# lh3/miniasm

Hardware: AMD Instinct MI355X
Metric: PAF overlaps processed/sec (hit-filter->trans-reduce->GFA) (higher is better)
Workload: dtype u32

## Files before the change

include/mahip.h:

```cpp
#ifndef MAHIP_H
#define MAHIP_H

#include <stddef.h>
#include <stdint.h>
#include "miniasm_amd.h"

#ifdef __cplusplus
extern "C" {
#endif

typedef struct mahip_ctx mahip_ctx_t;

int mahip_device_count(void);
mahip_ctx_t *mahip_create(int device, void *stream);
void mahip_destroy(mahip_ctx_t *c);
const char *mahip_strerror(void);
int mahip_sync(mahip_ctx_t *c);
int mahip_first_launch(mahip_ctx_t *c);

int mahip_hits_upload(mahip_ctx_t *c, const ma_hit_t *h, size_t n, uint32_t n_seq);
int mahip_hits_adopt(mahip_ctx_t *c, const void *d_hits, size_t n, uint32_t n_seq);
int mahip_set_shard(mahip_ctx_t *c, uint32_t q_beg, uint32_t q_end);
int mahip_hits_balance(mahip_ctx_t *c, int world, uint32_t *bounds);
int mahip_set_shard_bounds(mahip_ctx_t *c, const uint32_t *bounds, int world);
// ... 114 lines not shown
int mahip_map_download(mahip_ctx_t *c, int32_t *map);
uint32_t mahip_n_seq_new(mahip_ctx_t *c);
int mahip_survivors_download(mahip_ctx_t *c, uint32_t *old_ids);
size_t mahip_hits_live(mahip_ctx_t *c);
int mahip_hits_download(mahip_ctx_t *c, ma_hit_t *out, size_t *n);

int mahip_sg_gen(mahip_ctx_t *c, const ma_opt_t *opt, int use_sub, const uint32_t *seq_len, const uint8_t *seq_del, uint32_t *n_arc);
int mahip_asg_upload(mahip_ctx_t *c, const asg_t *g);
int mahip_asg_del_trans(mahip_ctx_t *c, int fuzz, uint32_t *n_reduced);
int mahip_asg_symm(mahip_ctx_t *c, uint32_t *n_multi, uint32_t *n_asymm);
int mahip_asg_del_multi(mahip_ctx_t *c, uint32_t *n_multi);
int mahip_asg_del_asymm(mahip_ctx_t *c, uint32_t *n_asymm);
int mahip_asg_del_short(mahip_ctx_t *c, float drop_ratio, uint32_t *n_short);
int mahip_asg_squeeze(mahip_ctx_t *c);
int mahip_tail_handoff(mahip_ctx_t *from, mahip_ctx_t *to);
int mahip_asg_cut_tip(mahip_ctx_t *c, int max_ext, uint32_t *n_cut);
int mahip_asg_cut_internal(mahip_ctx_t *c, int max_ext, uint32_t *n_cut);
int mahip_asg_cut_biloop(mahip_ctx_t *c, int max_ext, uint32_t *n_cut);
int mahip_asg_pop_bubble(mahip_ctx_t *c, int max_dist, uint32_t *n_pop, uint32_t *n_tips);
uint32_t mahip_bubble_seq_sweeps(mahip_ctx_t *c);
enum { MAHIP_BUBBLE_TIERS = 5, MAHIP_BUBBLE_THREAD = 1, MAHIP_BUBBLE_WAVE_LDS = 2, MAHIP_BUBBLE_WAVE_HBM = 3 };
typedef struct { uint32_t n_iter, max_tier, seq_sweep, form[MAHIP_BUBBLE_TIERS]; uint64_t n_src[MAHIP_BUBBLE_TIERS]; } mahip_clean_info_t;
int mahip_clean_last(mahip_ctx_t *c, mahip_clean_info_t *out);
int mahip_ug_gen(mahip_ctx_t *c, uint32_t *n_utg, uint32_t *n_members, uint32_t *n_uarc);
int mahip_ug_download(mahip_ctx_t *c, uint32_t *u_n, uint32_t *u_len, uint32_t *u_start, uint32_t *u_end, uint32_t *u_off, uint64_t *members, asg_arc_t *uarcs);
typedef struct { uint64_t src_off, dst_off; uint32_t src_len, len; uint32_t rev, pad; } mahip_useq_job_t;
int mahip_useq_begin(mahip_ctx_t *c, size_t arena_bytes);
int mahip_useq_batch(mahip_ctx_t *c, const char *h_seq, size_t seq_bytes, const mahip_useq_job_t *h_jobs, size_t n_jobs);
int mahip_useq_end(mahip_ctx_t *c, char *h_arena);
enum { MAHIP_FASTX_OK = 0, MAHIP_FASTX_CR, MAHIP_FASTX_FIRST_BYTE, MAHIP_FASTX_FASTA_LINE_START, MAHIP_FASTX_FASTQ_SHAPE, MAHIP_FASTX_FASTQ_QUAL_LEN, MAHIP_FASTX_TOO_MANY_LINES,
// ... 268 lines not shown
```

miniasm_amd/csrc/graph.hip:

```cpp
#include "mahip_internal.hpp"
#include <type_traits>

#define DEAD 0x80000000u
#define ADEL 0x80000000u

struct HitColsG { const uint32_t *qid, *qs, *qe, *tn, *ts, *te, *ml, *bl; };
struct ArcCols { uint32_t *u, *v, *len, *ol; };

static HitColsG gcols_of(mahip_ctx *c)
{
	HitColsG h;
	h.qid = P<uint32_t>(c->col[0]); h.qs = P<uint32_t>(c->col[1]); h.qe = P<uint32_t>(c->col[2]); h.tn = P<uint32_t>(c->col[3]);
	h.ts = P<uint32_t>(c->col[4]); h.te = P<uint32_t>(c->col[5]); h.ml = P<uint32_t>(c->col[6]); h.bl = P<uint32_t>(c->col[7]);
	return h;
}
static ArcCols arcs_of(mahip_ctx *c, int g)
{
	ArcCols a;
	a.u = P<uint32_t>(c->au[g]); a.v = P<uint32_t>(c->av[g]); a.len = P<uint32_t>(c->alen[g]); a.ol = P<uint32_t>(c->aol[g]);
	return a;
}
static int reserve_arcs(mahip_ctx *c, size_t n)
{
	for (int g = 0; g < 2; ++g) {
// ... 897 lines not shown
	c->n_arc = n_out;
	c->arcs_clean = true;
	if (index_mode > 0 || (index_mode == 0 && changed)) CHK(arc_reindex(c));
	return 0;
}


extern "C" int mahip_sg_flags(mahip_ctx_t *c, const ma_opt_t *opt, int use_sub, const uint32_t *seq_len, const uint8_t *seq_del)
{
	HIPCHK(hipSetDevice(c->dev));
	CHK(hits_need_cols(c, "mahip_sg_gen"));
	size_t n = c->n_hits;
	uint32_t R = c->n_seq;
	CHK(dev_reserve(c, c->slen, ((size_t)R + 4) * 4)); CHK(dev_reserve(c, c->sdel, (size_t)R + 16));
	c->sg_max_hang = opt->max_hang; c->sg_int_frac = opt->int_frac; c->sg_min_ovlp = opt->min_ovlp;
	c->gsq = false; c->arcs_clean = false;
	CHK(ctr_zero(c));
	unsigned long long *ctr = P<unsigned long long>(c->ctr);
	const uint32_t *d_len = nullptr; const uint8_t *d_del = nullptr;
	if (seq_len) { CHK(dev_reserve(c, c->big0, ((size_t)R + 4) * 4)); HIPCHK(hipMemcpyAsync(c->big0.p, seq_len, (size_t)R * 4, hipMemcpyHostToDevice, c->st)); d_len = P<uint32_t>(c->big0); }
	if (seq_del) { CHK(dev_reserve(c, c->big1, (size_t)R + 16)); HIPCHK(hipMemcpyAsync(c->big1.p, seq_del, R, hipMemcpyHostToDevice, c->st)); d_del = P<uint8_t>(c->big1); }
	if (!use_sub && !d_len) { mahip_set_error("mahip_sg_gen: need sub or seq_len"); return -1; }
	if (R) hipLaunchKernelGGL(k_sg_seq, dim3(grid_for(R, 256)), dim3(256), 0, c->st, use_sub ? (const uint2*)P<uint2>(c->sub[0]) : (const uint2*)nullptr,
	                          c->has_map ? (const uint8_t*)P<uint8_t>(c->r_del) : (const uint8_t*)nullptr, d_len, d_del, R, P<uint32_t>(c->slen), P<uint8_t>(c->sdel));
	c->ag = 0;
	if (n) CHK(dev_reserve(c, c->sgmask, (n / 64 + 8) * 8));
	if (n) {
		ProfScope ps(c, "k_sg_arcs", 64.0 * (double)c->n_live);
		hipLaunchKernelGGL(k_sg_arcs, dim3(grid_for(n, 256, MA_STREAM_BLOCKS)), dim3(256), 0, c->st, gcols_of(c), n, (const uint32_t*)P<uint32_t>(c->slen), P<uint8_t>(c->sdel),
		                   opt->max_hang, opt->int_frac, opt->min_ovlp, ctr,
		                   c->lazy_squeeze ? (const uint8_t*)P<uint8_t>(c->r_del) : (const uint8_t*)nullptr, P<unsigned long long>(c->sgmask));
// ... 376 lines not shown
		HIPCHK(hipMemcpyAsync(c->slen.p, c->big0.p, (size_t)Rn * 4, hipMemcpyDeviceToDevice, c->st));
		HIPCHK(hipMemcpyAsync(c->sdel.p, c->big1.p, (size_t)Rn, hipMemcpyDeviceToDevice, c->st));
		HIPCHK(hipMemcpyAsync(c->idx.p, c->pos.p, 2 * (size_t)Rn * 8, hipMemcpyDeviceToDevice, c->st));
	}
	HIPCHK(hipGetLastError());
	c->gsq = true;
	return 0;
}

__global__ __launch_bounds__(256) void k_sub_squeeze_g(const uint2 *__restrict__ sub, const int32_t *__restrict__ map, uint32_t n_seq, uint2 *__restrict__ out)
{
	uint32_t r = blockIdx.x * 256 + threadIdx.x;
	if (r < n_seq && map[r] >= 0) out[map[r]] = sub[r];
}

extern "C" int mahip_tail_handoff(mahip_ctx_t *s, mahip_ctx_t *d)
{
	if (s == d || s->dev != d->dev) { mahip_set_error("mahip_tail_handoff: two contexts on one device"); return -1; }
	HIPCHK(hipSetDevice(s->dev));
	if (!s->graph_ready) { mahip_set_error("mahip_tail_handoff: no graph"); return -1; }
	CHK(mahip_asg_squeeze(s));
	const uint32_t Rn = s->has_map ? s->n_seq_new : s->n_seq;
	const size_t n = s->n_arc;
	const bool have_sub = s->sub[0].p != nullptr && s->n_seq > 0;
	CHK(reserve_arcs(d, n));
	CHK(dev_reserve(d, d->slen, ((size_t)Rn + 4) * 4)); CHK(dev_reserve(d, d->sdel, (size_t)Rn + 16));
	CHK(dev_reserve(d, d->idx, (2 * (size_t)Rn + 2) * 8));
	CHK(dev_reserve(d, d->sub[0], ((size_t)Rn + 1) * 8)); CHK(dev_reserve(d, d->surv, ((size_t)Rn + 1) * 4));
	if (n) {
		HIPCHK(hipMemcpyAsync(d->au[0].p, s->au[s->ag].p, n * 4, hipMemcpyDeviceToDevice, s->st));
		HIPCHK(hipMemcpyAsync(d->av[0].p, s->av[s->ag].p, n * 4, hipMemcpyDeviceToDevice, s->st));
		HIPCHK(hipMemcpyAsync(d->alen[0].p, s->alen[s->ag].p, n * 4, hipMemcpyDeviceToDevice, s->st));
		HIPCHK(hipMemcpyAsync(d->aol[0].p, s->aol[s->ag].p, n * 4, hipMemcpyDeviceToDevice, s->st));
	}
	if (Rn) {
		HIPCHK(hipMemcpyAsync(d->slen.p, s->slen.p, (size_t)Rn * 4, hipMemcpyDeviceToDevice, s->st));
		HIPCHK(hipMemcpyAsync(d->sdel.p, s->sdel.p, (size_t)Rn, hipMemcpyDeviceToDevice, s->st));
		HIPCHK(hipMemcpyAsync(d->idx.p, s->idx.p, 2 * (size_t)Rn * 8, hipMemcpyDeviceToDevice, s->st));
		if (have_sub) {
			if (s->has_map) hipLaunchKernelGGL(k_sub_squeeze_g, dim3(grid_for(s->n_seq, 256)), dim3(256), 0, s->st, (const uint2*)P<uint2>(s->sub[0]), (const int32_t*)P<int32_t>(s->map), s->n_seq, P<uint2>(d->sub[0]));
			else HIPCHK(hipMemcpyAsync(d->sub[0].p, s->sub[0].p, (size_t)Rn * 8, hipMemcpyDeviceToDevice, s->st));
		}
		if (s->has_map || s->surv_ready) HIPCHK(hipMemcpyAsync(d->surv.p, s->surv.p, (size_t)Rn * 4, hipMemcpyDeviceToDevice, s->st));
	}
	HIPCHK(hipGetLastError());
	HIPCHK(hipStreamSynchronize(s->st));
	d->n_seq = Rn; d->n_seq_new = Rn; d->has_map = false; d->surv_ready = s->has_map || s->surv_ready; d->gsq = true; d->lazy_squeeze = false;
	d->soa_ready = false; d->gather_pending = false; d->sorted_here = false; d->n_hits = 0; d->n_live = 0;
	d->ag = 0; d->n_arc = (uint32_t)n; d->graph_ready = true;
	d->arcs_clean = s->arcs_clean;
	d->tie = s->tie;
	return 0;
}

extern "C" int mahip_asg_cleanup(mahip_ctx_t *c, uint32_t *n_arc)
{
	HIPCHK(hipSetDevice(c->dev));
	if (!c->graph_ready) { mahip_set_error("mahip_asg_cleanup: no graph"); return -1; }
	CHK(ctr_zero(c));
	CHK(arc_cleanup(c, c->n_arc, 0, 0));
	if (n_arc) *n_arc = c->n_arc;
	return 0;
}

// ... 170 lines not shown
```

miniasm_amd/csrc/hits.hip:

```cpp
#include "mahip_internal.hpp"

#define COL_QID 0
#define COL_QS 1
#define COL_QE 2
#define COL_TN 3
#define COL_TS 4
#define COL_TE 5
#define COL_ML 6
#define COL_BL 7
#define DEAD 0x80000000u

__global__ __launch_bounds__(256) void k_hit_keys(const ma_hit_t *__restrict__ h, size_t n, uint64_t *__restrict__ key,
                                                   uint32_t *__restrict__ val, uint32_t *__restrict__ keep, unsigned long long *__restrict__ ctr,
                                                   uint32_t q_beg, uint32_t q_end, int bi, int full)
{
	uint32_t cnt = 0;
	for (size_t i = (size_t)blockIdx.x * 256 + threadIdx.x; i < n; i += (size_t)gridDim.x * 256) {
		uint64_t k = h[i].qns;
		uint32_t q = (uint32_t)(k >> 32);
		int in = q >= q_beg && q < q_end;
		cnt += in;
		if (full) key[i] = k, val[i] = (uint32_t)i;
		else key[i] = (uint64_t)q << bi | i;
		if (keep) keep[i] = in;
// ... 860 lines not shown
static int reserve_read_arrays(mahip_ctx *c)
{
	size_t R = c->n_seq;
	CHK(dev_reserve(c, c->goff, (R + 2) * 4));
	for (int k = 0; k < 2; ++k) CHK(dev_reserve(c, c->sub[k], (R + 1) * 8));
	CHK(dev_reserve(c, c->r_cont, R + 16)); CHK(dev_reserve(c, c->r_used, R + 16));
	CHK(dev_reserve(c, c->r_del, R + 16)); CHK(dev_reserve(c, c->r_live, R + 16));
	CHK(dev_reserve(c, c->map, (R + 1) * 4));
	CHK(dev_reserve(c, c->surv, (R + 1) * 4));
	return 0;
}

static int hits_common_setup(mahip_ctx *c, size_t n, uint32_t n_seq)
{
	c->n_hits = n; c->n_in = n; c->n_live = n; c->n_seq = n_seq; c->n_seq_new = n_seq;
	c->soa_ready = false; c->has_map = false; c->surv_ready = false; c->graph_ready = false; c->gather_pending = false;
	c->hint_max_qs = 0; c->run_stride = 0; c->gk_runs = false; c->n_runs = 0;
	c->lazy_squeeze = false;
	c->sorted_here = false; c->hrank_ready = false; c->orank_ready = false;
	c->n_total = 0;
	c->shard_bounds.clear();
	memset(&c->tie, 0, sizeof(c->tie));
	CHK(reserve_read_arrays(c));
	for (int k = 0; k < 8; ++k) CHK(dev_reserve(c, c->col[k], (n + 128) * 4));
	return 0;
}

extern "C" int mahip_hits_upload(mahip_ctx_t *c, const ma_hit_t *h, size_t n, uint32_t n_seq)
{
	HIPCHK(hipSetDevice(c->dev));
	CHK(hits_common_setup(c, n, n_seq));
// ... 1016 lines not shown
```

miniasm_amd/csrc/mahip_api.hip:

```cpp
#include "mahip_internal.hpp"
#include <stdarg.h>

static thread_local char g_err[1024] = "";

void mahip_set_error(const char *fmt, ...)
{
	va_list ap;
	va_start(ap, fmt);
	vsnprintf(g_err, sizeof(g_err), fmt, ap);
	va_end(ap);
}

extern "C" const char *mahip_strerror(void) { return g_err; }

extern "C" int mahip_device_count(void)
{
	int n = 0;
	if (hipGetDeviceCount(&n) != hipSuccess) return 0;
	return n;
}

static bool pool_on() { static int v = -1; if (v < 0) { const char *e = getenv("MA_DEV_POOL"); v = !(e && atoi(e) == 0); } return v != 0; }

static std::mutex g_reg_mu;
static std::vector<mahip_ctx*> g_ctxs;
static void ctx_register(mahip_ctx *c) { std::lock_guard<std::mutex> g(g_reg_mu); g_ctxs.push_back(c); }
static void ctx_unregister(mahip_ctx *c)
{
	std::lock_guard<std::mutex> g(g_reg_mu);
	for (size_t i = 0; i < g_ctxs.size(); ++i) if (g_ctxs[i] == c) { g_ctxs[i] = g_ctxs.back(); g_ctxs.pop_back(); break; }
}

static DevPool::Base *pool_base_of(DevPool &P, const char *p)
{
	for (DevPool::Base &b : P.bases) if (p >= b.p && p < b.p + b.bytes) return &b;
	return nullptr;
}

static void pool_give_back(mahip_ctx *c, char *p, size_t cap)
{
	DevPool &P = c->pool;
	std::lock_guard<std::mutex> g(P.mu);
	DevPool::Base *base = pool_base_of(P, p);
	if (!base) { (void)hipFree(p); return; }
	DevPool::Piece nw = { p, cap, base->p };
	for (size_t i = 0; i < P.free_pieces.size();) {
		DevPool::Piece &f = P.free_pieces[i];
		if (f.base == nw.base && (f.p + f.cap == nw.p || nw.p + nw.cap == f.p)) {
			if (f.p < nw.p) nw.p = f.p;
			nw.cap += f.cap;
			P.free_pieces[i] = P.free_pieces.back(); P.free_pieces.pop_back();
			i = 0;
		} else ++i;
	}
	P.free_pieces.push_back(nw);
}

static size_t pool_trim_locked(DevPool &P)
{
	size_t freed = 0;
	for (size_t i = 0; i < P.free_pieces.size();) {
		const DevPool::Piece f = P.free_pieces[i];
		DevPool::Base *b = pool_base_of(P, f.p);
		if (b && f.p == b->p && f.cap == b->bytes) {
			(void)hipFree(b->p);
			freed += b->bytes;
			*b = P.bases.back(); P.bases.pop_back();
			P.free_pieces[i] = P.free_pieces.back(); P.free_pieces.pop_back();
		} else ++i;
	}
	return freed;
}
static size_t pool_trim(mahip_ctx *c) { std::lock_guard<std::mutex> g(c->pool.mu); return pool_trim_locked(c->pool); }
static void pool_trim_siblings(mahip_ctx *c)
{
	std::lock_guard<std::mutex> g(g_reg_mu);
	for (mahip_ctx *o : g_ctxs) if (o != c && o->dev == c->dev) (void)pool_trim(o);
}
static size_t pool_idle_bytes(mahip_ctx *c)
{
	std::lock_guard<std::mutex> g(c->pool.mu);
	size_t n = 0;
	for (const DevPool::Piece &f : c->pool.free_pieces) n += f.cap;
	return n;
}

static int pool_take(mahip_ctx *c, size_t want, void **out, size_t *cap)
{
	DevPool &P = c->pool;
	{
		std::lock_guard<std::mutex> g(P.mu);
		size_t best = (size_t)-1;
		for (size_t i = 0; i < P.free_pieces.size(); ++i)
			if (P.free_pieces[i].cap >= want && (best == (size_t)-1 || P.free_pieces[i].cap < P.free_pieces[best].cap)) best = i;
		if (best != (size_t)-1) {
			DevPool::Piece &f = P.free_pieces[best];
			*out = f.p;
			if (f.cap - want >= ((size_t)1 << 20)) { *cap = want; f.p += want; f.cap -= want; }
			else { *cap = f.cap; P.free_pieces[best] = P.free_pieces.back(); P.free_pieces.pop_back(); }
			return 0;
		}
	}
	void *p = nullptr;
	hipError_t e = hipMalloc(&p, want);
	if (e != hipSuccess) { (void)hipGetLastError(); (void)hipStreamSynchronize(c->st); (void)pool_trim(c); e = hipMalloc(&p, want); }
	if (e != hipSuccess) { (void)hipGetLastError(); pool_trim_siblings(c); e = hipMalloc(&p, want); }
	if (e != hipSuccess) { (void)hipGetLastError(); mahip_set_error("hipMalloc(%zu bytes) failed: %s (%zu bytes in use by this context)", want, hipGetErrorString(e), c->mem_bytes); return -1; }
	std::lock_guard<std::mutex> g(P.mu);
	P.bases.push_back({ (char*)p, want });
	*out = p; *cap = want;
	return 0;
}

void dev_pool_destroy(mahip_ctx *c)
{
	std::lock_guard<std::mutex> g(c->pool.mu);
	for (DevPool::Base &b : c->pool.bases) (void)hipFree(b.p);
	c->pool.bases.clear(); c->pool.free_pieces.clear();
}

int dev_reserve(mahip_ctx *c, DevBuf &b, size_t bytes)
{
	if (bytes <= b.cap) return 0;
	if (b.p) { HIPCHK(hipStreamSynchronize(c->st)); dev_free(c, b); }
	size_t want = (bytes + 255) & ~(size_t)255;
	if (pool_on()) {
		if (pool_take(c, want, &b.p, &b.cap) != 0) { b.p = nullptr; b.cap = 0; return -1; }
	} else {
		hipError_t e = hipMalloc(&b.p, want);
		if (e != hipSuccess) { (void)hipGetLastError(); b.p = nullptr; mahip_set_error("hipMalloc(%zu bytes) failed: %s", want, hipGetErrorString(e)); return -1; }
		b.cap = want;
	}
	c->mem_bytes += b.cap;
	return 0;
}

void dev_free(mahip_ctx *c, DevBuf &b)
{
	if (b.p) {
		c->mem_bytes -= b.cap;
		if (pool_on()) {
			if (b.ext) (void)hipDeviceSynchronize();
			pool_give_back(c, (char*)b.p, b.cap);
		} else (void)hipFree(b.p);
	}
	b.p = nullptr; b.cap = 0; b.ext = false;
}

extern "C" int mahip_mem_trim(mahip_ctx_t *c, size_t *released)
{
	HIPCHK(hipSetDevice(c->dev));
	HIPCHK(hipStreamSynchronize(c->st));
	const size_t n = pool_trim(c);
	if (released) *released = n;
	return 0;
}
extern "C" size_t mahip_mem_pool_bytes(mahip_ctx_t *c) { return pool_idle_bytes(c); }

int ctr_zero(mahip_ctx *c)
{
	HIPCHK(hipMemsetAsync(c->ctr.p, 0, CT_STICKY * 8, c->st));
// ... 81 lines not shown
	closedir(dp);
}

extern "C" mahip_ctx_t *mahip_create(int device, void *stream)
{
	int n = 0;
	hipError_t e = hipGetDeviceCount(&n);
	if (e != hipSuccess || n <= 0) {
		mahip_set_error("mahip_create: no HIP device available (%s); this library has no CPU fallback", e == hipSuccess ? "device count 0" : hipGetErrorString(e));
		return nullptr;
	}
	if (device < 0 || device >= n) { mahip_set_error("mahip_create: device %d out of range (0..%d)", device, n - 1); return nullptr; }
	if (hipSetDevice(device) != hipSuccess) { mahip_set_error("mahip_create: hipSetDevice(%d) failed", device); return nullptr; }
	pin_to_gpu_node(device);
	mahip_ctx *c = new mahip_ctx();
	c->dev = device;
	ctx_register(c);
	if (stream) c->st = (hipStream_t)stream, c->own_stream = false;
	else {
		if (hipStreamCreateWithFlags(&c->st, hipStreamNonBlocking) != hipSuccess) { mahip_set_error("mahip_create: hipStreamCreate failed"); ctx_unregister(c); delete c; return nullptr; }
		c->own_stream = true;
	}
	if (dev_reserve(c, c->ctr, CT_ALLOC_WORDS * 8) != 0) { ctx_unregister(c); delete c; return nullptr; }
	if (hipHostMalloc((void**)&c->h_ctr, 72 * 8, hipHostMallocCoherent | hipHostMallocMapped) != hipSuccess) { mahip_set_error("mahip_create: hipHostMalloc failed"); ctx_unregister(c); delete c; return nullptr; }
	memset(c->h_ctr, 0, 72 * 8);
	if (hipMemsetAsync(c->ctr.p, 0, CT_ALLOC_WORDS * 8, c->st) != hipSuccess) { mahip_set_error("mahip_create: memset failed"); ctx_unregister(c); delete c; return nullptr; }
	{ const char *s = getenv("MA_EXACT_TIES"); c->tie_mode = s == 0 || *s == 0 ? 2 : atoi(s) != 0 ? 1 : 0; }
	return c;
}

extern "C" void mahip_destroy(mahip_ctx_t *c)
{
	if (!c) return;
	ctx_unregister(c);
	(void)hipSetDevice(c->dev);
	(void)hipStreamSynchronize(c->st);
	for (auto &e : c->pev) { (void)hipEventDestroy(e.a); (void)hipEventDestroy(e.b); }
	for (hipEvent_t e : c->mark_ev) if (e) (void)hipEventDestroy(e);
	for (hipEvent_t e : c->sub_ev) if (e) (void)hipEventDestroy(e);
	for (hipStream_t t : c->sub_side) if (t) (void)hipStreamDestroy(t);
	DevBuf *all[] = { &c->aos_own, &c->goff, &c->sub[0], &c->sub[1], &c->r_cont, &c->r_used, &c->r_del, &c->r_live, &c->map, &c->surv,
		&c->au[0], &c->au[1], &c->av[0], &c->av[1], &c->alen[0], &c->alen[1], &c->aol[0], &c->aol[1], &c->idx, &c->sdel, &c->slen,
		&c->keep, &c->pos, &c->gs_tmp, &c->key[0], &c->key[1], &c->val[0], &c->val[1], &c->hist, &c->scan_tmp[0], &c->scan_tmp[1], &c->scan_tmp[2],
		&c->ctr, &c->ovf, &c->big0, &c->big1, &c->marks, &c->sgmask, &c->sidx, &c->hrank, &c->orank, &c->aslot, &c->apos, &c->pushrows[0], &c->pushrows[1], &c->xb[0], &c->xb[1], &c->gpos, &c->tdig, &c->wantb, &c->wseg };
	for (DevBuf *b : all) dev_free(c, *b);
	for (int k = 0; k < 8; ++k) dev_free(c, c->col[k]);
	c->hwalk.drop(); c->hdig.drop();
	mahip_comm_destroy(c);
	paf_free(c);
	clean_free(c);
	ug_free(c);
	useq_free(c);
	text_free(c);
	xfer_pool_free(c);
	free(c->gzip_rows);
	free(c->gzip_members);
	dev_pool_destroy(c);
	if (c->h_ctr) (void)hipHostFree(c->h_ctr);
	if (c->own_stream) (void)hipStreamDestroy(c->st);
	delete c;
}
// ... 119 lines not shown
```

miniasm_amd/csrc/mahip_internal.hpp:

```cpp
#pragma once
#include <hip/hip_runtime.h>
#include <stdint.h>
#include <stdio.h>
#include <stdlib.h>
#include <string.h>
#include <time.h>
#include <vector>
#include <mutex>
#include <string>
#include "mahip.h"
#include "ma_core.h"

void mahip_set_error(const char *fmt, ...);
extern "C" int ma_timing_level(void);

#define HIPCHK(expr) do { hipError_t e_ = (expr); if (e_ != hipSuccess) { \
	mahip_set_error("%s:%d: %s -> %s", __FILE__, __LINE__, #expr, hipGetErrorString(e_)); return -1; } } while (0)
#define CHK(expr) do { int r_ = (expr); if (r_ != 0) return r_; } while (0)

struct DevBuf {
	void *p = nullptr;
	size_t cap = 0;
	bool ext = false;
};

struct ProfEvent { const char *name; hipEvent_t a, b; double alg_bytes; };
struct ProfAcc { const char *name; uint64_t launches; double ms; double alg_bytes; };

struct DevPool {
	struct Base { char *p; size_t bytes; };
	struct Piece { char *p; size_t cap; char *base; };
	std::vector<Base> bases;
	std::vector<Piece> free_pieces;
	std::mutex mu;
};

struct BigHost { void *p = nullptr; size_t bytes = 0; bool mapped = false; bool reserve(size_t n); void drop(); };

struct mahip_ctx {
	int dev = 0;
	hipStream_t st = nullptr;
	bool own_stream = false;
	size_t mem_bytes = 0;
	DevPool pool;

	size_t n_hits = 0;
	size_t n_in = 0;
	bool full_input = true;
	DevBuf gpos;
	uint64_t n_total = 0;
	size_t n_live = 0;
	uint32_t n_seq = 0;
	uint32_t q_beg = 0, q_end = 0xffffffffu;
	std::vector<uint32_t> shard_bounds;
	uint32_t hint_max_qs = 0;
	uint32_t paf_max_qs = 0;
	const ma_hit_t *d_aos = nullptr;
	DevBuf aos_own;
	DevBuf col[8];
	DevBuf goff;
	DevBuf sub[2];
	DevBuf r_cont, r_used, r_del, r_live;
	DevBuf map;
	DevBuf surv;
	bool soa_ready = false, has_map = false, lazy_squeeze = false;
	bool surv_ready = false;
	int sg_max_hang = 0, sg_min_ovlp = 0; float sg_int_frac = 0;
	int tie_mode = 2;
	DevBuf sidx;
	DevBuf hrank;
	DevBuf orank;
	DevBuf aslot;
	DevBuf apos;
	DevBuf pushrows[2];
	uint32_t n_push = 0;
	bool sorted_here = false, hrank_ready = false, orank_ready = false;
	bool gather_pending = false; int gk_gen = 0, gk_bi = 0;
	bool gk_runs = false; size_t n_runs = 0; int run_stride = 0;
	bool push_ordered = false;
	mahip_tie_info_t tie = {0, 0, 0, 0, 0, 0, 0, 0, 0};
	uint32_t n_seq_new = 0;

	DevBuf au[2], av[2], alen[2], aol[2];
	int ag = 0;
	uint32_t n_arc = 0;
	DevBuf idx;
	DevBuf sdel;
	DevBuf slen;
	bool graph_ready = false;
	bool gsq = false;
	void *comm = nullptr;
	DevBuf xb[2];
	void *clean = nullptr;
	void *ug = nullptr;
	void *useq = nullptr;
	void *text = nullptr;

	DevBuf keep, pos;
	BigHost hwalk, hdig;
	DevBuf tdig;
	DevBuf wantb;
	DevBuf wseg;
	DevBuf key[2], val[2];
	DevBuf hist;
	DevBuf scan_tmp[3];
	DevBuf gs_tmp;
	DevBuf ctr;
	DevBuf ovf;
	DevBuf big0, big1;
	DevBuf marks;
	DevBuf sgmask;
	uint64_t *h_ctr = nullptr;
	unsigned long long ctr_seq = 0;
	uint32_t scan_ticket = 0, scan_epoch = 0;
	void *xfer = nullptr;
	mahip_xfer_info_t xfer_last = {};
	void *paf = nullptr;
	bool paf_keep_odd = false;
	mahip_bgzf_info_t bgzf_last = {};
	mahip_gzip_info_t gzip_last = {};
	mahip_gzip_item_t *gzip_rows = nullptr;
	uint64_t gzip_n_rows = 0;
	mahip_gzip_members_info_t gzip_mlast = {0, 0, 0, -1, 0, {0, 0}};
	mahip_gzip_member_t *gzip_members = nullptr;
	uint64_t gzip_n_members = 0;

	hipEvent_t mark_ev[64] = {};
	hipStream_t sub_side[2] = {}; hipEvent_t sub_ev[3] = {};
	uint64_t scan_forms[3] = {0, 0, 0};
	mahip_sort_info_t sort_last = {};
	struct { int n_pass, bits[16], shift[16]; uint32_t fixed7; int groups; } rs_last = {};
	uint64_t tr_inner = 0;
	bool arcs_clean = false;
	bool radix_arcs = false;
	bool sub_fork_failed = false;
	unsigned long long mark_set = 0;
	bool prof = false;
	std::vector<ProfEvent> pev;
	std::vector<size_t> pstack;
	std::vector<ProfAcc> pacc;
};

int dev_reserve(mahip_ctx *c, DevBuf &b, size_t bytes);
void dev_free(mahip_ctx *c, DevBuf &b);
void prof_begin(mahip_ctx *c, const char *name, double alg_bytes);
void prof_end(mahip_ctx *c);
int prof_collect(mahip_ctx *c);
void prof_patch_last(mahip_ctx *c, const char *name, double alg_bytes);

struct ProfScope {
	mahip_ctx *c;
	ProfScope(mahip_ctx *c_, const char *name, double alg_bytes) : c(c_) { if (c->prof) prof_begin(c, name, alg_bytes); }
	~ProfScope() { if (c->prof) prof_end(c); }
};

// ... 295 lines not shown
```

miniasm_amd/host/pipeline.c:

```c
#define _GNU_SOURCE
#include <stdio.h>
#include <stdlib.h>
#include <pthread.h>
#include <string.h>
#include "ma_host.h"

#define GPU(call) do { if ((call) != 0) ma_gpu_fail(__func__); } while (0)

FILE *ma_log_fp = 0;
static const char *g_reads_fn = 0;
void ma_set_reads_file(const char *fn) { g_reads_fn = fn; }

void ma_set_log_path(const char *path)
{
	if (ma_log_fp && ma_log_fp != stderr) fclose(ma_log_fp);
	ma_log_fp = path && *path ? fopen(path, "w") : 0;
}

static void print_subs(const sdict_t *d, const ma_sub_t *sub, FILE *out)
{
	uint32_t i;
	for (i = 0; i < d->n_seq; ++i)
		if (!d->seq[i].del && sub[i].s != sub[i].e)
			fprintf(out, "%s\t%d\t%d\n", d->seq[i].name, sub[i].s, sub[i].e);
// ... 28 lines not shown
	for (i = 0; i < n; ++i) memcpy(blob + off[i], view->seq[i].name, off[i + 1] - off[i]);
	rc = mahip_text_names(c, blob, off, n, del);
	free(blob); free(off); free(del);
	return rc;
}

static const char *text_reason(int reason)
{
	return reason == MAHIP_TEXT_SWITCHED_OFF ? "MA_TEXT_DEVICE is not 1" : reason == MAHIP_TEXT_NOMEM ? "no memory for its buffers" : reason == MAHIP_TEXT_NO_NAMES ? "the names are not on the device" :
	       reason == MAHIP_TEXT_NO_UG ? "no unitigs on the device" : reason == MAHIP_TEXT_NO_SEQ ? "no finished sequence arena in this context" : reason == MAHIP_TEXT_SEQ_NUL ? "a NUL byte in the sequences" :
	       reason == MAHIP_TEXT_TOO_MANY ? "too many records" : "ok";
}

static int text_sink_file(void *arg, const char *p, size_t n) { return fwrite(p, 1, n, (FILE*)arg) == n ? 0 : -1; }

int ma_pipeline_head(mahip_ctx_t *c, const ma_opt_t *opt, const sdict_t *d, const char *outfmt, int stage, int flags, uint32_t st[4])
{
	int no_first = flags & 1, no_second = flags & 2, have_sub = 0, squeezed = 0;
	size_t n_hits = 0, n_rem = 0;
	uint32_t R = d->n_seq, n_seq_new = R, n_red = 0;
	float cov = 40.0f;
	FILE *lg = MA_LOG;

	const int graph_out = strcmp(outfmt, "ug") == 0 || strcmp(outfmt, "sg") == 0;
	const int fused = !no_first && !no_second && stage >= 5 && graph_out && !getenv("MA_NO_FUSE");
	size_t n_cont_hits = 0;

	const int ht = ma_timing_level() >= 2;
	double ht0 = sys_realtime();
#define HT(label) do { if (ht) { mahip_sync(c); fprintf(stderr, "[T::head] %-28s %8.3f ms\n", label, (sys_realtime() - ht0) * 1e3); ht0 = sys_realtime(); } } while (0)
	GPU(mahip_hits_sort(c));
	HT("sort");
	if (fused) {
		size_t n_cut = 0, n_flt = 0, n_rem2 = 0;
		fprintf(lg, "[M::%s] ===> Step 2: 1-pass (crude) read selection <===\n", "main");
		GPU(mahip_hits_sub(c, opt->min_dp, opt->min_iden, 0, 0, &n_rem));
		HT("sub #1");
		if (ma_verbose >= 3) fprintf(lg, "[M::%s::%s] %ld query sequences remain after sub\n", "ma_hit_sub", sys_timestamp(), (long)n_rem);
		GPU(mahip_hits_cutflt_sub(c, 0, opt->min_span, (int)(opt->max_hang * 1.5), (int)(opt->min_ovlp * .5), opt->min_dp, opt->min_iden, opt->min_span / 2,
		                          1, &n_cut, &n_flt, &cov, &n_rem2));
		HT("cut+flt+sub #2");
// ... 30 lines not shown
			GPU(mahip_hits_sub(c, opt->min_dp, opt->min_iden, opt->min_span / 2, slot, &n_rem));
			if (ma_verbose >= 3) fprintf(lg, "[M::%s::%s] %ld query sequences remain after sub\n", "ma_hit_sub", sys_timestamp(), (long)n_rem);
			GPU(mahip_hits_cut(c, slot, opt->min_span, &n_hits));
			if (ma_verbose >= 3) fprintf(lg, "[M::%s::%s] %ld hits remain after cut\n", "ma_hit_cut", sys_timestamp(), (long)n_hits);
			if (!no_first) GPU(mahip_sub_merge(c));
			have_sub = 1;
		}
		if (stage >= 5 && have_sub) {
			GPU(mahip_hits_contained(c, opt, 0, &n_seq_new, &n_hits));
			squeezed = 1;
			if (ma_verbose >= 3) fprintf(lg, "[M::%s::%s] %d sequences and %ld hits remain after containment removal\n", "ma_hit_contained", sys_timestamp(), n_seq_new, (long)n_hits);
		}
	}
	}
	st[0] = have_sub, st[1] = squeezed, st[2] = 0, st[3] = 0;
	if (strcmp(outfmt, "ug") == 0 || strcmp(outfmt, "sg") == 0) {
		uint32_t n_arc = 0, *len = 0, r;
		uint8_t *sdel = 0;
		if (!fused) fprintf(lg, "[M::%s] ===> Step 4: graph cleaning <===\n", "main");
		if (!have_sub) {
			len = (uint32_t*)malloc((R ? R : 1) * 4);
			for (r = 0; r < R; ++r) len[r] = d->seq[r].len;
		}
		if (!squeezed) {
			sdel = (uint8_t*)malloc(R ? R : 1);
			for (r = 0; r < R; ++r) sdel[r] = d->seq[r].del;
		}
		GPU(mahip_sg_gen(c, opt, have_sub, len, sdel, &n_arc));
		HT("sg_gen");
		if (ma_timing_level() >= 1) {
			mahip_tie_info_t ti;
// ... 12 lines not shown
		}
		fprintf(lg, "[M::%s] read %d arcs\n", "ma_sg_gen", n_arc);
		if (stage >= 6) {
			fprintf(lg, "[M::%s] ===> Step 4.1: transitive reduction <===\n", "main");
			GPU(mahip_asg_del_trans(c, opt->gap_fuzz, &n_red));
			HT("del_trans");
			fprintf(lg, "[M::%s] transitively reduced %d arcs\n", "asg_arc_del_trans", n_red);
			if (n_red) {
				uint32_t n_multi = 0, n_asymm = 0;
				GPU(mahip_asg_symm(c, &n_multi, &n_asymm));
				HT("symm");
				fprintf(lg, "[M::%s] removed %d multi-arcs\n", "asg_arc_del_multi", n_multi);
				fprintf(lg, "[M::%s] removed %d asymmetric arcs\n", "asg_arc_del_asymm", n_asymm);
			}
		}
		st[2] = n_red, st[3] = 1;
	}
	return 0;
}

static int dev_cut_tip(mahip_ctx_t *c, int max_ext)
{
	uint32_t n = 0;
	GPU(mahip_asg_cut_tip(c, max_ext, &n));
	fprintf(MA_LOG, "[M::%s] cut %d tips\n", "asg_cut_tip", n);
	return (int)n;
}
static int dev_pop_bubble(mahip_ctx_t *c, int max_dist)
{
	uint32_t n = 0, t = 0;
	GPU(mahip_asg_pop_bubble(c, max_dist, &n, &t));
	fprintf(MA_LOG, "[M::%s] popped %d bubbles and trimmed %d tips\n", "asg_pop_bubble", n, t);
	return (int)n;
}
// ... 86 lines not shown
	uint32_t k;
	for (k = v->lo; k < v->hi; ++k) v->dst[k] = v->src[v->old[k]], v->dst[k].del = 0, v->dst[k].aux = 0;
	return 0;
}

static int tail_text_prepare(ma_tail_job_t *j, mahip_ctx_t *c, int kind);
static int tail_text_prepare_ug(ma_tail_job_t *j, mahip_ctx_t *c, const asg_arc_t *links, uint32_t n_links, int with_seq);

ma_tail_job_t *ma_pipeline_tail_fetch(mahip_ctx_t *c, const ma_opt_t *opt, const sdict_t *d, const char *outfmt, int stage, const uint32_t st[4])
{
	ma_tail_job_t *j = (ma_tail_job_t*)calloc(1, sizeof(ma_tail_job_t));
	const uint32_t R = d->n_seq;
	j->opt = *opt; j->d = d; j->stage = stage; j->ctx = c;
	if (strlen(outfmt) < sizeof(j->outfmt)) strcpy(j->outfmt, outfmt);
	j->have_sub = st[0]; j->squeezed = st[1]; j->n_red = st[2]; j->have_graph = st[3];
	j->t_fetch[0] = sys_realtime();
	j->view.n_seq = R; j->view.seq = d->seq;
	if (j->squeezed) {
		uint32_t k, n_new = mahip_n_seq_new(c), *old = (uint32_t*)malloc((n_new ? n_new : 1) * 4);
		GPU(mahip_survivors_download(c, old));
		j->view.seq = (sd_seq_t*)ma_big_alloc(((size_t)n_new + 1) * sizeof(sd_seq_t));
		if (n_new < 200000) {
			for (k = 0; k < n_new; ++k) j->view.seq[k] = d->seq[old[k]], j->view.seq[k].del = 0, j->view.seq[k].aux = 0;
		} else {
			view_job_t vj[8];
			pthread_t th[8];
			int t, T = ma_ingest_threads(), ok[8];
			if (T > 8) T = 8;
			if (T < 1) T = 1;
			for (t = 0; t < T; ++t) { vj[t].dst = j->view.seq; vj[t].src = d->seq; vj[t].old = old; vj[t].lo = (uint32_t)((uint64_t)n_new * (uint64_t)t / (uint64_t)T); vj[t].hi = (uint32_t)((uint64_t)n_new * (uint64_t)(t + 1) / (uint64_t)T); }
// ... 255 lines not shown
```

Baseline: 6.600 billion.

## Defer graph build to tail by swapping per-batch device buffers between contexts

In the fused graph-output path, the head can now skip graph generation and transitive reduction and mark hits as pending. The tail handoff then swaps the whole per-batch buffer set (split out into a new CtxBatch base struct) into the receiving context instead of squeezing and copying a finished graph. The graph is built later, in tail fetch. To let buffers move between contexts, the device pool becomes a heap object with reference accounting that is freed once the last buffer is returned. The aim is to overlap the graph stage with the next batch's head work and avoid device-to-device copies, at the cost of more complex buffer ownership and extra stream syncs when a buffer is freed into a foreign pool.

```diff
diff --git a/include/mahip.h b/include/mahip.h
--- a/include/mahip.h
+++ b/include/mahip.h
@@ -152,6 +152,7 @@
 int mahip_asg_del_short(mahip_ctx_t *c, float drop_ratio, uint32_t *n_short);
 int mahip_asg_squeeze(mahip_ctx_t *c);
 int mahip_tail_handoff(mahip_ctx_t *from, mahip_ctx_t *to);
+int mahip_graph_defer(mahip_ctx_t *c);
 int mahip_asg_cut_tip(mahip_ctx_t *c, int max_ext, uint32_t *n_cut);
 int mahip_asg_cut_internal(mahip_ctx_t *c, int max_ext, uint32_t *n_cut);
 int mahip_asg_cut_biloop(mahip_ctx_t *c, int max_ext, uint32_t *n_cut);
diff --git a/miniasm_amd/csrc/graph.hip b/miniasm_amd/csrc/graph.hip
--- a/miniasm_amd/csrc/graph.hip
+++ b/miniasm_amd/csrc/graph.hip
@@ -935,7 +935,7 @@
 	uint32_t R = c->n_seq;
 	CHK(dev_reserve(c, c->slen, ((size_t)R + 4) * 4)); CHK(dev_reserve(c, c->sdel, (size_t)R + 16));
 	c->sg_max_hang = opt->max_hang; c->sg_int_frac = opt->int_frac; c->sg_min_ovlp = opt->min_ovlp;
-	c->gsq = false; c->arcs_clean = false;
+	c->gsq = false; c->arcs_clean = false; c->hits_pending = false;
 	CHK(ctr_zero(c));
 	unsigned long long *ctr = P<unsigned long long>(c->ctr);
 	const uint32_t *d_len = nullptr; const uint8_t *d_del = nullptr;
@@ -1342,10 +1342,44 @@
 	if (r < n_seq && map[r] >= 0) out[map[r]] = sub[r];
 }
 
+extern "C" int mahip_graph_defer(mahip_ctx_t *c)
+{
+	const bool sharded = c->q_beg > 0 || (c->n_seq && c->q_end < c->n_seq);
+	if (c->prof || sharded || !c->full_input || c->comm || c->graph_ready || !c->has_map || !(c->soa_ready || c->gather_pending)) return 0;
+	c->hits_pending = true;
+	return 1;
+}
+
+static int batch_exchange(mahip_ctx *s, mahip_ctx *d)
+{
+	const bool d_sharded = d->q_beg > 0 || (d->n_seq && d->q_end < d->n_seq);
+	if (d_sharded || !d->full_input || d->comm) { mahip_set_error("mahip_tail_handoff: the receiving context is a shard's: it cannot make the graph of a whole input"); return -1; }
+	{
+		std::vector<DevBuf*> sb, db;
+		s->each_buf([&sb](DevBuf &b) { sb.push_back(&b); });
+		d->each_buf([&db](DevBuf &b) { db.push_back(&b); });
+		for (size_t i = 0; i < sb.size(); ++i) if (db[i]->cap == 0 && sb[i]->cap) CHK(dev_reserve(d, *db[i], sb[i]->cap));
+	}
+	size_t bs = 0, bd = 0;
+	s->each_buf([&bs](DevBuf &b) { bs += b.cap; });
+	d->each_buf([&bd](DevBuf &b) { bd += b.cap; });
+	std::swap(static_cast<CtxBatch&>(*s), static_cast<CtxBatch&>(*d));
+	s->mem_bytes += bd; s->mem_bytes -= bs;
+	d->mem_bytes += bs; d->mem_bytes -= bd;
+	s->n_hits = s->n_in = s->n_live = 0; s->n_total = 0; s->d_aos = nullptr; s->shard_bounds.clear();
+	s->soa_ready = s->has_map = s->lazy_squeeze = s->surv_ready = false;
+	s->sorted_here = s->hrank_ready = s->orank_ready = false;
+	s->gather_pending = s->gk_runs = false; s->n_runs = 0; s->run_stride = 0; s->hint_max_qs = 0;
+	s->n_push = 0; s->push_ordered = false;
+	s->n_arc = 0; s->ag = 0; s->graph_ready = s->hits_pending = s->gsq = s->arcs_clean = false;
+	return 0;
+}
+
 extern "C" int mahip_tail_handoff(mahip_ctx_t *s, mahip_ctx_t *d)
 {
 	if (s == d || s->dev != d->dev) { mahip_set_error("mahip_tail_handoff: two contexts on one device"); return -1; }
 	HIPCHK(hipSetDevice(s->dev));
+	if (!s->graph_ready && s->hits_pending) return batch_exchange(s, d);
 	if (!s->graph_ready) { mahip_set_error("mahip_tail_handoff: no graph"); return -1; }
 	CHK(mahip_asg_squeeze(s));
 	const uint32_t Rn = s->has_map ? s->n_seq_new : s->n_seq;
@@ -1375,7 +1409,7 @@
 	HIPCHK(hipStreamSynchronize(s->st));
 	d->n_seq = Rn; d->n_seq_new = Rn; d->has_map = false; d->surv_ready = s->has_map || s->surv_ready; d->gsq = true; d->lazy_squeeze = false;
 	d->soa_ready = false; d->gather_pending = false; d->sorted_here = false; d->n_hits = 0; d->n_live = 0;
-	d->ag = 0; d->n_arc = (uint32_t)n; d->graph_ready = true;
+	d->ag = 0; d->n_arc = (uint32_t)n; d->graph_ready = true; d->hits_pending = false;
 	d->arcs_clean = s->arcs_clean;
 	d->tie = s->tie;
 	return 0;
diff --git a/miniasm_amd/csrc/hits.hip b/miniasm_amd/csrc/hits.hip
--- a/miniasm_amd/csrc/hits.hip
+++ b/miniasm_amd/csrc/hits.hip
@@ -898,7 +898,7 @@
 static int hits_common_setup(mahip_ctx *c, size_t n, uint32_t n_seq)
 {
 	c->n_hits = n; c->n_in = n; c->n_live = n; c->n_seq = n_seq; c->n_seq_new = n_seq;
-	c->soa_ready = false; c->has_map = false; c->surv_ready = false; c->graph_ready = false; c->gather_pending = false;
+	c->soa_ready = false; c->has_map = false; c->surv_ready = false; c->graph_ready = false; c->hits_pending = false; c->gather_pending = false;
 	c->hint_max_qs = 0; c->run_stride = 0; c->gk_runs = false; c->n_runs = 0;
 	c->lazy_squeeze = false;
 	c->sorted_here = false; c->hrank_ready = false; c->orank_ready = false;
diff --git a/miniasm_amd/csrc/mahip_api.hip b/miniasm_amd/csrc/mahip_api.hip
--- a/miniasm_amd/csrc/mahip_api.hip
+++ b/miniasm_amd/csrc/mahip_api.hip
@@ -37,12 +37,17 @@
 	return nullptr;
 }
 
-static void pool_give_back(mahip_ctx *c, char *p, size_t cap)
-{
-	DevPool &P = c->pool;
+static size_t pool_trim_locked(DevPool &P);
+
+static void pool_give_back(DevPool *Pp, char *p, size_t cap)
+{
+	DevPool &P = *Pp;
+	bool last = false;
+	{
 	std::lock_guard<std::mutex> g(P.mu);
 	DevPool::Base *base = pool_base_of(P, p);
 	if (!base) { (void)hipFree(p); return; }
+	P.out_bytes -= cap;
 	DevPool::Piece nw = { p, cap, base->p };
 	for (size_t i = 0; i < P.free_pieces.size();) {
 		DevPool::Piece &f = P.free_pieces[i];
@@ -54,6 +59,9 @@
 		} else ++i;
 	}
 	P.free_pieces.push_back(nw);
+	if (P.closed) { (void)pool_trim_locked(P); last = P.out_bytes == 0; }
+	}
+	if (last) delete Pp;
 }
 
 static size_t pool_trim_locked(DevPool &P)
@@ -71,7 +79,7 @@
 	}
 	return freed;
 }
-static size_t pool_trim(mahip_ctx *c) { std::lock_guard<std::mutex> g(c->pool.mu); return pool_trim_locked(c->pool); }
+static size_t pool_trim(mahip_ctx *c) { std::lock_guard<std::mutex> g(c->pool->mu); return pool_trim_locked(*c->pool); }
 static void pool_trim_siblings(mahip_ctx *c)
 {
 	std::lock_guard<std::mutex> g(g_reg_mu);
@@ -79,15 +87,15 @@
 }
 static size_t pool_idle_bytes(mahip_ctx *c)
 {
-	std::lock_guard<std::mutex> g(c->pool.mu);
+	std::lock_guard<std::mutex> g(c->pool->mu);
 	size_t n = 0;
-	for (const DevPool::Piece &f : c->pool.free_pieces) n += f.cap;
+	for (const DevPool::Piece &f : c->pool->free_pieces) n += f.cap;
 	return n;
 }
 
 static int pool_take(mahip_ctx *c, size_t want, void **out, size_t *cap)
 {
-	DevPool &P = c->pool;
+	DevPool &P = *c->pool;
 	{
 		std::lock_guard<std::mutex> g(P.mu);
 		size_t best = (size_t)-1;
@@ -98,6 +106,7 @@
 			*out = f.p;
 			if (f.cap - want >= ((size_t)1 << 20)) { *cap = want; f.p += want; f.cap -= want; }
 			else { *cap = f.cap; P.free_pieces[best] = P.free_pieces.back(); P.free_pieces.pop_back(); }
+			P.out_bytes += *cap;
 			return 0;
 		}
 	}
@@ -108,15 +117,23 @@
 	if (e != hipSuccess) { (void)hipGetLastError(); mahip_set_error("hipMalloc(%zu bytes) failed: %s (%zu bytes in use by this context)", want, hipGetErrorString(e), c->mem_bytes); return -1; }
 	std::lock_guard<std::mutex> g(P.mu);
 	P.bases.push_back({ (char*)p, want });
+	P.out_bytes += want;
 	*out = p; *cap = want;
 	return 0;
 }
 
 void dev_pool_destroy(mahip_ctx *c)
 {
-	std::lock_guard<std::mutex> g(c->pool.mu);
-	for (DevPool::Base &b : c->pool.bases) (void)hipFree(b.p);
-	c->pool.bases.clear(); c->pool.free_pieces.clear();
+	DevPool *P = c->pool;
+	bool last;
+	{
+		std::lock_guard<std::mutex> g(P->mu);
+		P->closed = true;
+		(void)pool_trim_locked(*P);
+		last = P->out_bytes == 0;
+	}
+	c->pool = nullptr;
+	if (last) delete P;
 }
 
 int dev_reserve(mahip_ctx *c, DevBuf &b, size_t bytes)
@@ -126,6 +143,7 @@
 	size_t want = (bytes + 255) & ~(size_t)255;
 	if (pool_on()) {
 		if (pool_take(c, want, &b.p, &b.cap) != 0) { b.p = nullptr; b.cap = 0; return -1; }
+		b.owner = c->pool;
 	} else {
 		hipError_t e = hipMalloc(&b.p, want);
 		if (e != hipSuccess) { (void)hipGetLastError(); b.p = nullptr; mahip_set_error("hipMalloc(%zu bytes) failed: %s", want, hipGetErrorString(e)); return -1; }
@@ -141,10 +159,11 @@
 		c->mem_bytes -= b.cap;
 		if (pool_on()) {
 			if (b.ext) (void)hipDeviceSynchronize();
-			pool_give_back(c, (char*)b.p, b.cap);
+			else if (b.owner != c->pool) (void)hipStreamSynchronize(c->st);
+			pool_give_back(b.owner, (char*)b.p, b.cap);
 		} else (void)hipFree(b.p);
 	}
-	b.p = nullptr; b.cap = 0; b.ext = false;
+	b.p = nullptr; b.cap = 0; b.ext = false; b.owner = nullptr;
 }
 
 extern "C" int mahip_mem_trim(mahip_ctx_t *c, size_t *released)
@@ -256,17 +275,18 @@
 	if (hipSetDevice(device) != hipSuccess) { mahip_set_error("mahip_create: hipSetDevice(%d) failed", device); return nullptr; }
 	pin_to_gpu_node(device);
 	mahip_ctx *c = new mahip_ctx();
+	c->pool = new DevPool();
 	c->dev = device;
 	ctx_register(c);
 	if (stream) c->st = (hipStream_t)stream, c->own_stream = false;
 	else {
-		if (hipStreamCreateWithFlags(&c->st, hipStreamNonBlocking) != hipSuccess) { mahip_set_error("mahip_create: hipStreamCreate failed"); ctx_unregister(c); delete c; return nullptr; }
+		if (hipStreamCreateWithFlags(&c->st, hipStreamNonBlocking) != hipSuccess) { mahip_set_error("mahip_create: hipStreamCreate failed"); ctx_unregister(c); delete c->pool; delete c; return nullptr; }
 		c->own_stream = true;
 	}
-	if (dev_reserve(c, c->ctr, CT_ALLOC_WORDS * 8) != 0) { ctx_unregister(c); delete c; return nullptr; }
-	if (hipHostMalloc((void**)&c->h_ctr, 72 * 8, hipHostMallocCoherent | hipHostMallocMapped) != hipSuccess) { mahip_set_error("mahip_create: hipHostMalloc failed"); ctx_unregister(c); delete c; return nullptr; }
+	if (dev_reserve(c, c->ctr, CT_ALLOC_WORDS * 8) != 0) { ctx_unregister(c); delete c->pool; delete c; return nullptr; }
+	if (hipHostMalloc((void**)&c->h_ctr, 72 * 8, hipHostMallocCoherent | hipHostMallocMapped) != hipSuccess) { mahip_set_error("mahip_create: hipHostMalloc failed"); ctx_unregister(c); delete c->pool; delete c; return nullptr; }
 	memset(c->h_ctr, 0, 72 * 8);
-	if (hipMemsetAsync(c->ctr.p, 0, CT_ALLOC_WORDS * 8, c->st) != hipSuccess) { mahip_set_error("mahip_create: memset failed"); ctx_unregister(c); delete c; return nullptr; }
+	if (hipMemsetAsync(c->ctr.p, 0, CT_ALLOC_WORDS * 8, c->st) != hipSuccess) { mahip_set_error("mahip_create: memset failed"); ctx_unregister(c); delete c->pool; delete c; return nullptr; }
 	{ const char *s = getenv("MA_EXACT_TIES"); c->tie_mode = s == 0 || *s == 0 ? 2 : atoi(s) != 0 ? 1 : 0; }
 	return c;
 }
@@ -281,12 +301,8 @@
 	for (hipEvent_t e : c->mark_ev) if (e) (void)hipEventDestroy(e);
 	for (hipEvent_t e : c->sub_ev) if (e) (void)hipEventDestroy(e);
 	for (hipStream_t t : c->sub_side) if (t) (void)hipStreamDestroy(t);
-	DevBuf *all[] = { &c->aos_own, &c->goff, &c->sub[0], &c->sub[1], &c->r_cont, &c->r_used, &c->r_del, &c->r_live, &c->map, &c->surv,
-		&c->au[0], &c->au[1], &c->av[0], &c->av[1], &c->alen[0], &c->alen[1], &c->aol[0], &c->aol[1], &c->idx, &c->sdel, &c->slen,
-		&c->keep, &c->pos, &c->gs_tmp, &c->key[0], &c->key[1], &c->val[0], &c->val[1], &c->hist, &c->scan_tmp[0], &c->scan_tmp[1], &c->scan_tmp[2],
-		&c->ctr, &c->ovf, &c->big0, &c->big1, &c->marks, &c->sgmask, &c->sidx, &c->hrank, &c->orank, &c->aslot, &c->apos, &c->pushrows[0], &c->pushrows[1], &c->xb[0], &c->xb[1], &c->gpos, &c->tdig, &c->wantb, &c->wseg };
-	for (DevBuf *b : all) dev_free(c, *b);
-	for (int k = 0; k < 8; ++k) dev_free(c, c->col[k]);
+	c->each_buf([c](DevBuf &b) { dev_free(c, b); });
+	c->each_own_buf([c](DevBuf &b) { dev_free(c, b); });
 	c->hwalk.drop(); c->hdig.drop();
 	mahip_comm_destroy(c);
 	paf_free(c);
diff --git a/miniasm_amd/csrc/mahip_internal.hpp b/miniasm_amd/csrc/mahip_internal.hpp
--- a/miniasm_amd/csrc/mahip_internal.hpp
+++ b/miniasm_amd/csrc/mahip_internal.hpp
@@ -18,10 +18,12 @@
 	mahip_set_error("%s:%d: %s -> %s", __FILE__, __LINE__, #expr, hipGetErrorString(e_)); return -1; } } while (0)
 #define CHK(expr) do { int r_ = (expr); if (r_ != 0) return r_; } while (0)
 
+struct DevPool;
 struct DevBuf {
 	void *p = nullptr;
 	size_t cap = 0;
 	bool ext = false;
+	DevPool *owner = nullptr;
 };
 
 struct ProfEvent { const char *name; hipEvent_t a, b; double alg_bytes; };
@@ -33,28 +35,21 @@
 	std::vector<Base> bases;
 	std::vector<Piece> free_pieces;
 	std::mutex mu;
+	size_t out_bytes = 0;
+	bool closed = false;
 };
 
 struct BigHost { void *p = nullptr; size_t bytes = 0; bool mapped = false; bool reserve(size_t n); void drop(); };
 
-struct mahip_ctx {
-	int dev = 0;
-	hipStream_t st = nullptr;
-	bool own_stream = false;
-	size_t mem_bytes = 0;
-	DevPool pool;
-
+struct CtxBatch {
 	size_t n_hits = 0;
 	size_t n_in = 0;
-	bool full_input = true;
 	DevBuf gpos;
 	uint64_t n_total = 0;
 	size_t n_live = 0;
 	uint32_t n_seq = 0;
-	uint32_t q_beg = 0, q_end = 0xffffffffu;
 	std::vector<uint32_t> shard_bounds;
 	uint32_t hint_max_qs = 0;
-	uint32_t paf_max_qs = 0;
 	const ma_hit_t *d_aos = nullptr;
 	DevBuf aos_own;
 	DevBuf col[8];
@@ -66,7 +61,6 @@
 	bool soa_ready = false, has_map = false, lazy_squeeze = false;
 	bool surv_ready = false;
 	int sg_max_hang = 0, sg_min_ovlp = 0; float sg_int_frac = 0;
-	int tie_mode = 2;
 	DevBuf sidx;
 	DevBuf hrank;
 	DevBuf orank;
@@ -80,6 +74,7 @@
 	bool push_ordered = false;
 	mahip_tie_info_t tie = {0, 0, 0, 0, 0, 0, 0, 0, 0};
 	uint32_t n_seq_new = 0;
+	mahip_sort_info_t sort_last = {};
 
 	DevBuf au[2], av[2], alen[2], aol[2];
 	int ag = 0;
@@ -88,7 +83,43 @@
 	DevBuf sdel;
 	DevBuf slen;
 	bool graph_ready = false;
+	bool hits_pending = false;
 	bool gsq = false;
+	uint64_t tr_inner = 0;
+	bool arcs_clean = false;
+
+	DevBuf keep, pos;
+	BigHost hwalk, hdig;
+	DevBuf tdig;
+	DevBuf wantb;
+	DevBuf wseg;
+	DevBuf key[2], val[2];
+	DevBuf ovf;
+	DevBuf big0, big1;
+	DevBuf marks;
+	DevBuf sgmask;
+
+	template <class F> void each_buf(F f)
+	{
+		DevBuf *all[] = { &gpos, &aos_own, &goff, &sub[0], &sub[1], &r_cont, &r_used, &r_del, &r_live, &map, &surv, &sidx, &hrank, &orank, &aslot, &apos, &pushrows[0], &pushrows[1],
+			&au[0], &au[1], &av[0], &av[1], &alen[0], &alen[1], &aol[0], &aol[1], &idx, &sdel, &slen, &keep, &pos, &tdig, &wantb, &wseg, &key[0], &key[1], &val[0], &val[1],
+			&ovf, &big0, &big1, &marks, &sgmask };
+		for (DevBuf *b : all) f(*b);
+		for (int k = 0; k < 8; ++k) f(col[k]);
+	}
+};
+
+struct mahip_ctx : CtxBatch {
+	int dev = 0;
+	hipStream_t st = nullptr;
+	bool own_stream = false;
+	size_t mem_bytes = 0;
+	DevPool *pool = nullptr;
+
+	bool full_input = true;
+	uint32_t q_beg = 0, q_end = 0xffffffffu;
+	uint32_t paf_max_qs = 0;
+	int tie_mode = 2;
 	void *comm = nullptr;
 	DevBuf xb[2];
 	void *clean = nullptr;
@@ -96,20 +127,10 @@
 	void *useq = nullptr;
 	void *text = nullptr;
 
-	DevBuf keep, pos;
-	BigHost hwalk, hdig;
-	DevBuf tdig;
-	DevBuf wantb;
-	DevBuf wseg;
-	DevBuf key[2], val[2];
 	DevBuf hist;
 	DevBuf scan_tmp[3];
 	DevBuf gs_tmp;
 	DevBuf ctr;
-	DevBuf ovf;
-	DevBuf big0, big1;
-	DevBuf marks;
-	DevBuf sgmask;
 	uint64_t *h_ctr = nullptr;
 	unsigned long long ctr_seq = 0;
 	uint32_t scan_ticket = 0, scan_epoch = 0;
@@ -128,10 +149,7 @@
 	hipEvent_t mark_ev[64] = {};
 	hipStream_t sub_side[2] = {}; hipEvent_t sub_ev[3] = {};
 	uint64_t scan_forms[3] = {0, 0, 0};
-	mahip_sort_info_t sort_last = {};
 	struct { int n_pass, bits[16], shift[16]; uint32_t fixed7; int groups; } rs_last = {};
-	uint64_t tr_inner = 0;
-	bool arcs_clean = false;
 	bool radix_arcs = false;
 	bool sub_fork_failed = false;
 	unsigned long long mark_set = 0;
@@ -139,6 +157,12 @@
 	std::vector<ProfEvent> pev;
 	std::vector<size_t> pstack;
 	std::vector<ProfAcc> pacc;
+
+	template <class F> void each_own_buf(F f)
+	{
+		DevBuf *all[] = { &xb[0], &xb[1], &hist, &scan_tmp[0], &scan_tmp[1], &scan_tmp[2], &gs_tmp, &ctr };
+		for (DevBuf *b : all) f(*b);
+	}
 };
 
 int dev_reserve(mahip_ctx *c, DevBuf &b, size_t bytes);
diff --git a/miniasm_amd/host/pipeline.c b/miniasm_amd/host/pipeline.c
--- a/miniasm_amd/host/pipeline.c
+++ b/miniasm_amd/host/pipeline.c
@@ -66,17 +66,18 @@
 
 static int text_sink_file(void *arg, const char *p, size_t n) { return fwrite(p, 1, n, (FILE*)arg) == n ? 0 : -1; }
 
+static uint32_t head_graph(mahip_ctx_t *c, const ma_opt_t *opt, const sdict_t *d, const char *outfmt, int stage, int have_sub, int squeezed, int fused);
+
 int ma_pipeline_head(mahip_ctx_t *c, const ma_opt_t *opt, const sdict_t *d, const char *outfmt, int stage, int flags, uint32_t st[4])
 {
 	int no_first = flags & 1, no_second = flags & 2, have_sub = 0, squeezed = 0;
 	size_t n_hits = 0, n_rem = 0;
-	uint32_t R = d->n_seq, n_seq_new = R, n_red = 0;
+	uint32_t R = d->n_seq, n_seq_new = R;
 	float cov = 40.0f;
 	FILE *lg = MA_LOG;
 
 	const int graph_out = strcmp(outfmt, "ug") == 0 || strcmp(outfmt, "sg") == 0;
 	const int fused = !no_first && !no_second && stage >= 5 && graph_out && !getenv("MA_NO_FUSE");
-	size_t n_cont_hits = 0;
 
 	const int ht = ma_timing_level() >= 2;
 	double ht0 = sys_realtime();
@@ -137,7 +138,25 @@
 	}
 	}
 	st[0] = have_sub, st[1] = squeezed, st[2] = 0, st[3] = 0;
-	if (strcmp(outfmt, "ug") == 0 || strcmp(outfmt, "sg") == 0) {
+	if (graph_out) {
+		if (fused && !ht && mahip_graph_defer(c) == 1) { st[3] = 2; return 0; }
+		st[2] = head_graph(c, opt, d, outfmt, stage, have_sub, squeezed, fused), st[3] = 1;
+	}
+	return 0;
+}
+#undef HT
+
+static uint32_t head_graph(mahip_ctx_t *c, const ma_opt_t *opt, const sdict_t *d, const char *outfmt, int stage, int have_sub, int squeezed, int fused)
+{
+	const uint32_t R = d->n_seq, n_seq_new = squeezed ? mahip_n_seq_new(c) : R;
+	uint32_t n_red = 0;
+	size_t n_cont_hits = 0;
+	FILE *lg = MA_LOG;
+	const int ht = ma_timing_level() >= 2;
+	double ht0 = sys_realtime();
+#define HT(label) do { if (ht) { mahip_sync(c); fprintf(stderr, "[T::head] %-28s %8.3f ms\n", label, (sys_realtime() - ht0) * 1e3); ht0 = sys_realtime(); } } while (0)
+	(void)outfmt;
+	{
 		uint32_t n_arc = 0, *len = 0, r;
 		uint8_t *sdel = 0;
 		if (!fused) fprintf(lg, "[M::%s] ===> Step 4: graph cleaning <===\n", "main");
@@ -180,10 +199,10 @@
 				fprintf(lg, "[M::%s] removed %d asymmetric arcs\n", "asg_arc_del_asymm", n_asymm);
 			}
 		}
-		st[2] = n_red, st[3] = 1;
-	}
-	return 0;
-}
+	}
+	return n_red;
+}
+#undef HT
 
 static int dev_cut_tip(mahip_ctx_t *c, int max_ext)
 {
@@ -300,6 +319,10 @@
 	j->opt = *opt; j->d = d; j->stage = stage; j->ctx = c;
 	if (strlen(outfmt) < sizeof(j->outfmt)) strcpy(j->outfmt, outfmt);
 	j->have_sub = st[0]; j->squeezed = st[1]; j->n_red = st[2]; j->have_graph = st[3];
+	if (st[3] == 2) {
+		j->n_red = head_graph(c, opt, d, outfmt, stage, j->have_sub, j->squeezed, 1);
+		j->have_graph = 1;
+	}
 	j->t_fetch[0] = sys_realtime();
 	j->view.n_seq = R; j->view.seq = d->seq;
 	if (j->squeezed) {
```

New measurement: 6.489 billion. 1.7% lower.
